# NVIDIAGameWorks/kaolin-wisp

Measured on AMD Instinct MI355X. Metric: training rays/sec, HashGrid NeRF (nerf_hash.yaml), synthetic Lego 800x800, higher is better.
Workload: dtype bf16

## Files before the change

### kaolin-wisp_amd/csrc/render.hip

```cpp
#include "wisp_common.h"
#include "raygen_dev.h"

#define WISP_DPP_ADD(V, CTRL, RMASK)                                                                                  \
    V += __builtin_bit_cast(float, __builtin_amdgcn_update_dpp(0, __builtin_bit_cast(int, V), CTRL, RMASK, 0xf, false))
static __device__ __forceinline__ float wave_incl_scan_f(float v, int ) {
    WISP_DPP_ADD(v, 0x111, 0xf);
    WISP_DPP_ADD(v, 0x112, 0xf);
    WISP_DPP_ADD(v, 0x114, 0xf);
    WISP_DPP_ADD(v, 0x118, 0xf);
    WISP_DPP_ADD(v, 0x142, 0xa);
    WISP_DPP_ADD(v, 0x143, 0xc);
    return v;
}
#undef WISP_DPP_ADD

static __device__ __forceinline__ float wave_last_f(float v) {
    return __builtin_bit_cast(float, __builtin_amdgcn_readlane(__builtin_bit_cast(int, v), 63));
}

static __device__ __forceinline__ float wave_sum_f(float v) { return wave_last_f(wave_incl_scan_f(v, 0)); }

__global__ void __launch_bounds__(256)
packed_sum_reduce_kernel(const float* __restrict__ feats, int64_t s_total, int channels,
                         const int64_t* __restrict__ pack_starts, int64_t num_packs, float* __restrict__ out) {
    const int lane = threadIdx.x & 63;
    const int64_t p = (int64_t)blockIdx.x * (blockDim.x >> 6) + (threadIdx.x >> 6);
    if (p >= num_packs) return;
    const int64_t b = pack_starts[p], e = (p + 1 < num_packs) ? pack_starts[p + 1] : s_total;
    for (int c = 0; c < channels; ++c) {
        float acc = 0.0f;
        for (int64_t i = b + lane; i < e; i += 64) acc += feats[i * channels + c];
        acc = wave_sum_f(acc);
        if (lane == 0) out[p * channels + c] = acc;
    }
}

__global__ void __launch_bounds__(256)
packed_cumsum_kernel(const float* __restrict__ feats, int64_t s_total, int channels,
                     const int64_t* __restrict__ pack_starts, int64_t num_packs, int exclusive, int reverse,
                     float* __restrict__ out) {
    const int lane = threadIdx.x & 63;
    const int64_t p = (int64_t)blockIdx.x * (blockDim.x >> 6) + (threadIdx.x >> 6);
    if (p >= num_packs) return;
    const int64_t b = pack_starts[p], e = (p + 1 < num_packs) ? pack_starts[p + 1] : s_total;
    const int64_t len = e - b;
    for (int c = 0; c < channels; ++c) {
        float carry = 0.0f;
        for (int64_t k0 = 0; k0 < len; k0 += 64) {
            const int64_t k = k0 + lane;
            const int64_t i = reverse ? (e - 1 - k) : (b + k);
            const float v = (k < len) ? feats[i * channels + c] : 0.0f;
            const float inc = wave_incl_scan_f(v, lane);
            if (k < len) out[i * channels + c] = carry + (exclusive ? inc - v : inc);
            carry += wave_last_f(inc);
        }
    }
}

extern "C" int wisp_packed_sum_reduce(const float* feats, int64_t num_samples, int channels, const int64_t* pack_starts,
                                      int64_t num_packs, float* out, wisp_stream_t stream) {
    WISP_REQUIRE(num_samples >= 0 && num_packs >= 0 && channels >= 1, "bad sizes");
    if (num_packs == 0) return WISP_OK;
    WISP_REQUIRE(feats && pack_starts && out, "null pointer");
    hipLaunchKernelGGL(packed_sum_reduce_kernel, dim3((unsigned)ceil_div64(num_packs, 4)), dim3(256), 0,
                       (hipStream_t)stream, feats, num_samples, channels, pack_starts, num_packs, out);
    WISP_CHECK_LAUNCH();
    return WISP_OK;
}

extern "C" int wisp_packed_cumsum(const float* feats, int64_t num_samples, int channels, const int64_t* pack_starts,
                                  int64_t num_packs, int exclusive, int reverse, float* out, wisp_stream_t stream) {
    WISP_REQUIRE(num_samples >= 0 && num_packs >= 0 && channels >= 1, "bad sizes");
    if (num_packs == 0) return WISP_OK;
    WISP_REQUIRE(feats && pack_starts && out, "null pointer");
    hipLaunchKernelGGL(packed_cumsum_kernel, dim3((unsigned)ceil_div64(num_packs, 4)), dim3(256), 0,
                       (hipStream_t)stream, feats, num_samples, channels, pack_starts, num_packs, exclusive, reverse, out);
    WISP_CHECK_LAUNCH();
    return WISP_OK;
}

struct Bg { float r, g, b; };

#define PACK_WAVES 1

__global__ void __launch_bounds__(256)
composite_init_kernel(int64_t num_rays, Bg bg, float* __restrict__ rgb, float* __restrict__ alpha,
                      float* __restrict__ depth, uint8_t* __restrict__ hit) {
    const int64_t r = (int64_t)blockIdx.x * blockDim.x + threadIdx.x;
    if (r >= num_rays) return;
    rgb[r * 3] = bg.r; rgb[r * 3 + 1] = bg.g; rgb[r * 3 + 2] = bg.b;
    alpha[r] = 0.0f;
    if (depth) depth[r] = 0.0f;
    hit[r] = 0;
}

template <bool BY_RAY>
__global__ void __launch_bounds__(256)
composite_fwd_kernel(const float* __restrict__ color, const float* __restrict__ density,
                     const float* __restrict__ deltas, const float* __restrict__ depths,
                     const int64_t* __restrict__ ridx, const int64_t* __restrict__ pack_starts, int64_t num_packs,
                     int64_t s_total, Bg bg, float* __restrict__ out_rgb, float* __restrict__ out_alpha,
                     float* __restrict__ out_depth, uint8_t* __restrict__ out_hit, float* __restrict__ weights) {
    const int lane = threadIdx.x & 63;
    const int64_t p = (int64_t)blockIdx.x * (blockDim.x >> 6) + (threadIdx.x >> 6);
    if (p >= num_packs) return;
    const int64_t b = pack_starts[p], e = (BY_RAY || p + 1 < num_packs) ? pack_starts[p + 1] : s_total;
    if (BY_RAY && b == e) {
        if (lane == 0) {
            out_alpha[p] = 0.0f; out_hit[p] = 0;
            out_rgb[p * 3] = bg.r; out_rgb[p * 3 + 1] = bg.g; out_rgb[p * 3 + 2] = bg.b;
            if (out_depth) out_depth[p] = 0.0f;
        }
        return;
    }
    float carry = 0.0f, sr = 0.0f, sg = 0.0f, sb = 0.0f, sa = 0.0f, sd = 0.0f;
    for (int64_t k0 = b; k0 < e; k0 += 64) {
        const int64_t i = k0 + lane;
        const bool live = i < e;
        const float tau = live ? density[i] * deltas[i] : 0.0f;
        const float inc = wave_incl_scan_f(tau, lane);
        const float excl = carry + (inc - tau);
        carry += wave_last_f(inc);
        if (live) {
            const float T = expf(-excl);
            const float w = T * (1.0f - expf(-tau));
            weights[i] = w;
            sr += w * color[i * 3]; sg += w * color[i * 3 + 1]; sb += w * color[i * 3 + 2];
            sa += w;
            if (depths) sd += w * depths[i];
        }
    }
    sr = wave_sum_f(sr); sg = wave_sum_f(sg); sb = wave_sum_f(sb); sa = wave_sum_f(sa);
    if (depths) sd = wave_sum_f(sd);
    if (lane == 0) {
        const int64_t r = BY_RAY ? p : ridx[b];
        out_alpha[r] = sa;
        out_hit[r] = sa > 0.0f ? 1 : 0;
        const float om = 1.0f - sa;
        out_rgb[r * 3] = bg.r * om + sr; out_rgb[r * 3 + 1] = bg.g * om + sg; out_rgb[r * 3 + 2] = bg.b * om + sb;
        if (out_depth) out_depth[r] = sd;
    }
}

template <bool BY_RAY>
__global__ void __launch_bounds__(256)
composite_bwd_kernel(const float* __restrict__ grad_rgb, const float* __restrict__ grad_alpha,
                     const float* __restrict__ grad_depth, const float* __restrict__ color,
                     const float* __restrict__ density, const float* __restrict__ deltas,
                     const float* __restrict__ depths, const int64_t* __restrict__ ridx,
                     const int64_t* __restrict__ pack_starts, int64_t num_packs, int64_t s_total, Bg bg,
                     float* __restrict__ grad_color, float* __restrict__ grad_density) {
    const int lane = threadIdx.x & 63;
    const int64_t p = (int64_t)blockIdx.x * (blockDim.x >> 6) + (threadIdx.x >> 6);
    if (p >= num_packs) return;
    const int64_t b = pack_starts[p], e = (BY_RAY || p + 1 < num_packs) ? pack_starts[p + 1] : s_total;
    if (BY_RAY && b == e) return;
    const int64_t r = BY_RAY ? p : ridx[b];
    const float gr = grad_rgb[r * 3], gg = grad_rgb[r * 3 + 1], gb = grad_rgb[r * 3 + 2];
    const float ga = grad_alpha ? grad_alpha[r] : 0.0f;
    const float gd = (grad_depth && depths) ? grad_depth[r] : 0.0f;
    float carry = 0.0f, tot = 0.0f;
    for (int64_t k0 = b; k0 < e; k0 += 64) {
        const int64_t i = k0 + lane;
        const bool live = i < e;
        const float tau = live ? density[i] * deltas[i] : 0.0f;
        const float inc = wave_incl_scan_f(tau, lane);
        const float excl = carry + (inc - tau);
        carry += wave_last_f(inc);
        if (live) {
            const float w = expf(-excl) * (1.0f - expf(-tau));
            float G = gr * (color[i * 3] - bg.r) + gg * (color[i * 3 + 1] - bg.g) + gb * (color[i * 3 + 2] - bg.b) + ga;
            if (depths) G += gd * depths[i];
            tot += G * w;
        }
    }
    tot = wave_sum_f(tot);
    carry = 0.0f;
    float gcarry = 0.0f;
    for (int64_t k0 = b; k0 < e; k0 += 64) {
        const int64_t i = k0 + lane;
        const bool live = i < e;
        const float dl = live ? deltas[i] : 0.0f;
        const float tau = live ? density[i] * dl : 0.0f;
        const float inc = wave_incl_scan_f(tau, lane);
        const float excl = carry + (inc - tau);
        carry += wave_last_f(inc);
        float T = 0.0f, et = 0.0f, w = 0.0f, G = 0.0f;
        if (live) {
            T = expf(-excl); et = expf(-tau); w = T * (1.0f - et);
            G = gr * (color[i * 3] - bg.r) + gg * (color[i * 3 + 1] - bg.g) + gb * (color[i * 3 + 2] - bg.b) + ga;
            if (depths) G += gd * depths[i];
        }
        const float gw = G * w;
        const float ginc = wave_incl_scan_f(gw, lane);
        const float suffix = tot - (gcarry + ginc);
        gcarry += wave_last_f(ginc);
        if (live) {
            grad_color[i * 3] = w * gr; grad_color[i * 3 + 1] = w * gg; grad_color[i * 3 + 2] = w * gb;
            grad_density[i] = (G * T * et - suffix) * dl;
        }
    }
}

extern "C" int wisp_composite_fwd(const float* color, const float* density, const float* deltas, const float* depths,
                                  const int64_t* ridx, const int64_t* pack_starts, int64_t num_packs,
                                  int64_t num_samples, int64_t num_rays, const float* bg, float* out_rgb,
                                  float* out_alpha, float* out_depth, uint8_t* out_hit, float* weights,
                                  wisp_stream_t stream) {
    WISP_REQUIRE(num_rays >= 0 && num_packs >= 0 && num_samples >= 0, "bad sizes");
    WISP_REQUIRE(bg, "null bg");
    if (num_rays == 0) return WISP_OK;
    WISP_REQUIRE(out_rgb && out_alpha && out_hit, "null output");
    WISP_REQUIRE(out_depth == nullptr || depths != nullptr, "out_depth needs depths");
    hipStream_t s = (hipStream_t)stream;
    const Bg b{bg[0], bg[1], bg[2]};
    if (ridx == nullptr) {
        WISP_REQUIRE(pack_starts && num_packs == num_rays, "ray-offset mode needs offsets[R+1] and num_packs == num_rays");
        WISP_REQUIRE(num_samples == 0 || (color && density && deltas && weights), "null pointer");
        hipLaunchKernelGGL(composite_fwd_kernel<true>, dim3((unsigned)ceil_div64(num_rays, PACK_WAVES)), dim3(64 * PACK_WAVES), 0, s, color,
                           density, deltas, out_depth ? depths : nullptr, ridx, pack_starts, num_rays, num_samples, b,
                           out_rgb, out_alpha, out_depth, out_hit, weights);
        WISP_CHECK_LAUNCH();
        return WISP_OK;
    }
    hipLaunchKernelGGL(composite_init_kernel, dim3((unsigned)ceil_div64(num_rays, 256)), dim3(256), 0, s, num_rays, b,
                       out_rgb, out_alpha, out_depth, out_hit);
    if (num_packs > 0) {
        WISP_REQUIRE(color && density && deltas && ridx && pack_starts && weights, "null pointer");
        hipLaunchKernelGGL(composite_fwd_kernel<false>, dim3((unsigned)ceil_div64(num_packs, 4)), dim3(256), 0, s, color,
                           density, deltas, out_depth ? depths : nullptr, ridx, pack_starts, num_packs, num_samples, b,
                           out_rgb, out_alpha, out_depth, out_hit, weights);
    }
    WISP_CHECK_LAUNCH();
    return WISP_OK;
}

extern "C" int wisp_composite_bwd(const float* grad_rgb, const float* grad_alpha, const float* grad_depth,
                                  const float* color, const float* density, const float* deltas, const float* depths,
                                  const int64_t* ridx, const int64_t* pack_starts, int64_t num_packs,
                                  int64_t num_samples, const float* bg, float* grad_color, float* grad_density,
                                  wisp_stream_t stream) {
    WISP_REQUIRE(num_packs >= 0 && num_samples >= 0 && bg, "bad sizes");
    if (num_packs == 0) return WISP_OK;
    WISP_REQUIRE(grad_rgb && color && density && deltas && pack_starts && grad_color && grad_density, "null pointer");
    const Bg b{bg[0], bg[1], bg[2]};
    if (ridx == nullptr)
        hipLaunchKernelGGL(composite_bwd_kernel<true>, dim3((unsigned)ceil_div64(num_packs, PACK_WAVES)), dim3(64 * PACK_WAVES), 0,
                           (hipStream_t)stream, grad_rgb, grad_alpha, grad_depth, color, density, deltas, depths, ridx,
                           pack_starts, num_packs, num_samples, b, grad_color, grad_density);
    else
        hipLaunchKernelGGL(composite_bwd_kernel<false>, dim3((unsigned)ceil_div64(num_packs, 4)), dim3(256), 0,
                           (hipStream_t)stream, grad_rgb, grad_alpha, grad_depth, color, density, deltas, depths, ridx,
                           pack_starts, num_packs, num_samples, b, grad_color, grad_density);
    WISP_CHECK_LAUNCH();
    return WISP_OK;
}

__global__ void __launch_bounds__(256)
find_depth_bound_kernel(int64_t num_packs, int64_t num_nugs, const float* __restrict__ query,
                        const int32_t* __restrict__ curr_in, int32_t* __restrict__ curr_out,
                        const float* __restrict__ depth) {
    const int64_t t = (int64_t)blockIdx.x * blockDim.x + threadIdx.x;
    if (t >= num_packs) return;
    int32_t result = -1;
    const int32_t start = curr_in[t];
    if (start > -1) {
        uint32_t i = (uint32_t)start;
        uint32_t stop = (t == num_packs - 1) ? (uint32_t)num_packs : (uint32_t)curr_in[t + 1];
        if ((int64_t)stop > num_nugs) stop = (uint32_t)num_nugs;
        const float q = query[t];
        while (i < stop) {
            const float entry = depth[2 * (int64_t)i], exit_ = depth[2 * (int64_t)i + 1];
            if ((q >= entry && q <= exit_) || q < entry) { result = (int32_t)i; break; }
            ++i;
        }
    }
    curr_out[t] = result;
}

extern "C" int wisp_find_depth_bound(const float* query, const int32_t* curr_idxes, const float* nug_depth,
                                     int64_t num_packs, int64_t num_nugs, int32_t* out, wisp_stream_t stream) {
    WISP_REQUIRE(num_packs >= 0 && num_nugs >= 0, "bad sizes");
    if (num_packs == 0) return WISP_OK;
    WISP_REQUIRE(query && curr_idxes && nug_depth && out, "null pointer");
    hipLaunchKernelGGL(find_depth_bound_kernel, dim3((unsigned)ceil_div64(num_packs, 256)), dim3(256), 0, (hipStream_t)stream,
                       num_packs, num_nugs, query, curr_idxes, out, nug_depth);
    WISP_CHECK_LAUNCH();
    return WISP_OK;
}

__global__ void __launch_bounds__(256)
sphere_trace_step_kernel(int64_t num_packs, const float* __restrict__ nug_o, const float* __restrict__ nug_d,
                         const float* __restrict__ nug_depth, const int32_t* __restrict__ nug_pidx, float dist_max,
                         float thr_close, float thr_avg, float* __restrict__ t, const float* __restrict__ dist, float* __restrict__ dist_prev,
                         uint8_t* __restrict__ mask, uint8_t* __restrict__ hit, const int32_t* __restrict__ curr_in,
                         int32_t* __restrict__ curr_out, int64_t* __restrict__ curr_pidx, float* __restrict__ x) {
#pragma clang fp contract(off)
    const int64_t p = (int64_t)blockIdx.x * blockDim.x + threadIdx.x;
    if (p >= num_packs) return;
    const int32_t cur = curr_in[p];
    bool m = mask[p] != 0;
    bool h = hit[p] != 0;
    const float dd = dist[p];
    float tt = t[p] + dd;
    if (m) {
        h = fabsf(dd) < thr_close;
        h = h || (fabsf(dd + dist_prev[p]) * 0.5f < thr_avg);
        m = tt < dist_max;
    }
    m = m && !h;
    if (m) dist_prev[p] = dd;
    int32_t nxt = -1;
    if (cur > -1) {
        uint32_t i = (uint32_t)cur;
        const uint32_t stop = (p == num_packs - 1) ? (uint32_t)num_packs : (uint32_t)curr_in[p + 1];
        while (i < stop) {
            const float entry = nug_depth[2 * (int64_t)i], exit_ = nug_depth[2 * (int64_t)i + 1];
            if ((tt >= entry && tt <= exit_) || tt < entry) { nxt = (int32_t)i; break; }
            ++i;
        }
    }
    m = m && (nxt != -1);
    const bool jumped = nxt != cur;
    const int32_t now = m ? nxt : cur;
    if (m && jumped) tt = nug_depth[2 * (int64_t)now];
    if (m) {
        x[p * 3 + 0] = nug_o[p * 3 + 0] + nug_d[p * 3 + 0] * tt;
        x[p * 3 + 1] = nug_o[p * 3 + 1] + nug_d[p * 3 + 1] * tt;
        x[p * 3 + 2] = nug_o[p * 3 + 2] + nug_d[p * 3 + 2] * tt;
        curr_pidx[p] = (int64_t)nug_pidx[now];
    } else if (mask[p] != 0) {
        x[p * 3 + 0] = nug_o[p * 3 + 0] + nug_d[p * 3 + 0] * tt;
        x[p * 3 + 1] = nug_o[p * 3 + 1] + nug_d[p * 3 + 1] * tt;
        x[p * 3 + 2] = nug_o[p * 3 + 2] + nug_d[p * 3 + 2] * tt;
    }
    t[p] = tt;
    mask[p] = m ? 1 : 0;
    hit[p] = h ? 1 : 0;
    curr_out[p] = now;
}

extern "C" int wisp_sphere_trace_step(int64_t num_packs, const float* nug_o, const float* nug_d, const float* nug_depth,
                                      const int32_t* nug_pidx, float dist_max, float thr_close, float thr_avg, float* t,
                                      const float* dist,
                                      float* dist_prev, uint8_t* mask, uint8_t* hit, const int32_t* curr_in,
                                      int32_t* curr_out, int64_t* curr_pidx, float* x, wisp_stream_t stream) {
    WISP_REQUIRE(num_packs >= 0, "negative count");
    if (num_packs == 0) return WISP_OK;
    WISP_REQUIRE(nug_o && nug_d && nug_depth && nug_pidx && t && dist && dist_prev && mask && hit && curr_in && curr_out &&
                 curr_pidx && x, "null pointer");
    hipLaunchKernelGGL(sphere_trace_step_kernel, dim3((unsigned)ceil_div64(num_packs, 256)), dim3(256), 0, (hipStream_t)stream,
                       num_packs, nug_o, nug_d, nug_depth, nug_pidx, dist_max, thr_close, thr_avg, t, dist, dist_prev, mask, hit, curr_in,
                       curr_out, curr_pidx, x);
    WISP_CHECK_LAUNCH();
    return WISP_OK;
}

template <bool ORTHO>
__global__ void __launch_bounds__(256)
raygen_kernel(const float* __restrict__ pixel_x, const float* __restrict__ pixel_y, int64_t n, RayCam cam,
              float* __restrict__ origins, float* __restrict__ dirs) {
    const int64_t i = (int64_t)blockIdx.x * blockDim.x + threadIdx.x;
    if (i >= n) return;
    float ow[3], dn[3];
    wisp_camera_ray<ORTHO>(pixel_x[i], pixel_y[i], cam, ow, dn);
#pragma unroll
    for (int c = 0; c < 3; ++c) {
        origins[i * 3 + c] = ow[c];
        dirs[i * 3 + c] = dn[c];
    }
}

extern "C" int wisp_generate_rays(const float* pixel_x, const float* pixel_y, int64_t num_pixels, int ortho, float x0,
                                  float y0, float width, float height, float scale_x, float scale_y,
                                  const float* view_rotation, const float* view_translation, float* origins, float* dirs,
                                  wisp_stream_t stream) {
    WISP_REQUIRE(num_pixels >= 0, "negative count");
    if (num_pixels == 0) return WISP_OK;
    WISP_REQUIRE(pixel_x && pixel_y && view_rotation && view_translation && origins && dirs, "null pointer");
    WISP_REQUIRE(width > 0.0f && height > 0.0f, "bad image size");
    RayCam cam;
    cam.x0 = x0; cam.y0 = y0; cam.width = width; cam.height = height; cam.sx = scale_x; cam.sy = scale_y;
    for (int k = 0; k < 9; ++k) cam.r[k] = view_rotation[k];
    for (int k = 0; k < 3; ++k) cam.t[k] = view_translation[k];
    const dim3 grid((unsigned)ceil_div64(num_pixels, 256));
    if (ortho)
        hipLaunchKernelGGL(raygen_kernel<true>, grid, dim3(256), 0, (hipStream_t)stream, pixel_x, pixel_y, num_pixels, cam, origins, dirs);
    else
        hipLaunchKernelGGL(raygen_kernel<false>, grid, dim3(256), 0, (hipStream_t)stream, pixel_x, pixel_y, num_pixels, cam, origins, dirs);
    WISP_CHECK_LAUNCH();
    return WISP_OK;
}

#define LOSS_BLOCKS 256
__global__ void __launch_bounds__(256)
rgb_loss_kernel(const float* __restrict__ rgb, const float* __restrict__ gt, int64_t n, int kind, float inv_n,
                float* __restrict__ grad, float* __restrict__ partial) {
    __shared__ float part[4];
    float acc = 0.0f;
    for (int64_t i = (int64_t)blockIdx.x * 256 + threadIdx.x; i < n; i += (int64_t)gridDim.x * 256) {
        const float x = rgb[i] - gt[i];
        float l, g;
        if (kind == 0) { const float a = fabsf(x); l = a < 1.0f ? 0.5f * x * x : a - 0.5f; g = fminf(fmaxf(x, -1.0f), 1.0f); }
        else if (kind == 1) { l = x * x; g = 2.0f * x; }
        else { l = fabsf(x); g = (x > 0.0f) ? 1.0f : (x < 0.0f ? -1.0f : 0.0f); }
        acc += l;
        grad[i] = g * inv_n;
    }
#pragma unroll
    for (int off = 32; off > 0; off >>= 1) acc += __shfl_down(acc, off, 64);
    if ((threadIdx.x & 63) == 0) part[threadIdx.x >> 6] = acc;
    __syncthreads();
    if (threadIdx.x == 0) partial[blockIdx.x] = (part[0] + part[1]) + (part[2] + part[3]);
}

__global__ void __launch_bounds__(1024)
loss_sum_kernel(const float* __restrict__ partial, int n, float inv_n, float* __restrict__ loss) {
    __shared__ float part[16];
    float t = 0.0f;
    for (int base = 0; base < n; base += 8 * 1024) {
        float v[8];
#pragma unroll
        for (int k = 0; k < 8; ++k) { const int i = base + threadIdx.x + k * 1024; v[k] = i < n ? partial[i] : 0.0f; }
#pragma unroll
        for (int k = 0; k < 8; ++k) t += v[k];
    }
#pragma unroll
    for (int off = 32; off > 0; off >>= 1) t += __shfl_down(t, off, 64);
    if ((threadIdx.x & 63) == 0) part[threadIdx.x >> 6] = t;
    __syncthreads();
    if (threadIdx.x == 0) {
        float s = 0.0f;
#pragma unroll
        for (int w = 0; w < 16; ++w) s += part[w];
        loss[0] = s * inv_n;
    }
}

extern "C" int wisp_rgb_loss(const float* rgb, const float* gt, int64_t num_elements, int kind, float* grad, float* loss,
                             float* workspace, wisp_stream_t stream) {
    WISP_REQUIRE(num_elements > 0 && rgb && gt && grad && loss && workspace, "bad arguments");
    WISP_REQUIRE(kind >= 0 && kind <= 2, "kind: 0 huber, 1 l2, 2 l1");
    const int blocks = (int)min64(ceil_div64(num_elements, 256), LOSS_BLOCKS);
    const float inv_n = 1.0f / (float)num_elements;
    hipLaunchKernelGGL(rgb_loss_kernel, dim3(blocks), dim3(256), 0, (hipStream_t)stream, rgb, gt, num_elements, kind, inv_n, grad,
                       workspace + 1);
    hipLaunchKernelGGL(loss_sum_kernel, dim3(1), dim3(1024), 0, (hipStream_t)stream, workspace + 1, blocks, inv_n, loss);
    WISP_CHECK_LAUNCH();
    return WISP_OK;
}

template <int W>
__global__ void __launch_bounds__(64 * W)
composite_loss_kernel(const float* __restrict__ color, const float* __restrict__ density, const float* __restrict__ deltas,
                      const int64_t* __restrict__ offsets, int64_t num_rays, int groups, Bg bg, const float* __restrict__ gt, int kind,
                      float inv_n, float* __restrict__ grad_color, float* __restrict__ grad_density, float* __restrict__ out_rgb,
                      float* __restrict__ partial) {
    const int lane = threadIdx.x & 63;
    const int v = blockIdx.x * W + (threadIdx.x >> 6);
    if (v >= groups) return;
    float lacc = 0.0f;
    for (int64_t r = v; r < num_rays; r += groups) {
        const int64_t b = offsets[r], e = offsets[r + 1];
        const float gt0 = gt[r * 3], gt1 = gt[r * 3 + 1], gt2 = gt[r * 3 + 2];
        const bool single = e - b <= 64;
        float carry = 0.0f, sr = 0.0f, sg = 0.0f, sb = 0.0f, sa = 0.0f;
        float dl = 0.0f, T = 0.0f, et = 0.0f, w = 0.0f, c0 = 0.0f, c1 = 0.0f, c2 = 0.0f;
        for (int64_t k0 = b; k0 < e; k0 += 64) {
            const int64_t i = k0 + lane;
            const bool live = i < e;
            dl = live ? deltas[i] : 0.0f;
            const float dn = live ? density[i] : 0.0f;
            c0 = live ? color[i * 3] : 0.0f; c1 = live ? color[i * 3 + 1] : 0.0f; c2 = live ? color[i * 3 + 2] : 0.0f;
            const float tau = live ? dn * dl : 0.0f;
            const float inc = wave_incl_scan_f(tau, lane);
            const float excl = carry + (inc - tau);
            carry += wave_last_f(inc);
            T = 0.0f; et = 0.0f; w = 0.0f;
            if (live) {
                T = expf(-excl); et = expf(-tau);
                w = T * (1.0f - et);
                sr += w * c0; sg += w * c1; sb += w * c2;
                sa += w;
            }
        }
        if (b < e) { sr = wave_sum_f(sr); sg = wave_sum_f(sg); sb = wave_sum_f(sb); sa = wave_sum_f(sa); }
        const float om = 1.0f - sa;
        const float rgb[3] = {bg.r * om + sr, bg.g * om + sg, bg.b * om + sb};
        const float gtc[3] = {gt0, gt1, gt2};
        float g[3], lsum[3];
#pragma unroll
        for (int c = 0; c < 3; ++c) {
            const float x = rgb[c] - gtc[c];
            float l, d;
            if (kind == 0) { const float a = fabsf(x); l = a < 1.0f ? 0.5f * x * x : a - 0.5f; d = fminf(fmaxf(x, -1.0f), 1.0f); }
            else if (kind == 1) { l = x * x; d = 2.0f * x; }
            else { l = fabsf(x); d = (x > 0.0f) ? 1.0f : (x < 0.0f ? -1.0f : 0.0f); }
            lsum[c] = l;
            g[c] = d * inv_n;
        }
        lacc += (lsum[0] + lsum[1]) + lsum[2];
        if (out_rgb && lane == 0) { out_rgb[r * 3] = rgb[0]; out_rgb[r * 3 + 1] = rgb[1]; out_rgb[r * 3 + 2] = rgb[2]; }
        if (b == e) continue;
        const float gr = g[0], gg = g[1], gb = g[2];
        if (single) {
            const int64_t i = b + lane;
            const bool live = i < e;
            const float G = live ? gr * (c0 - bg.r) + gg * (c1 - bg.g) + gb * (c2 - bg.b) : 0.0f;
            const float gw = G * w;
            const float ginc = wave_incl_scan_f(gw, lane);
            const float tot = wave_last_f(ginc);
            const float suffix = tot - ginc;
            if (live) {
                grad_color[i * 3] = w * gr; grad_color[i * 3 + 1] = w * gg; grad_color[i * 3 + 2] = w * gb;
                grad_density[i] = (G * T * et - suffix) * dl;
            }
            continue;
        }
        carry = 0.0f;
        float tot = 0.0f;
        for (int64_t k0 = b; k0 < e; k0 += 64) {
            const int64_t i = k0 + lane;
            const bool live = i < e;
            const float tau = live ? density[i] * deltas[i] : 0.0f;
            const float inc = wave_incl_scan_f(tau, lane);
            const float excl = carry + (inc - tau);
            carry += wave_last_f(inc);
            if (live) {
                const float ww = expf(-excl) * (1.0f - expf(-tau));
                const float G = gr * (color[i * 3] - bg.r) + gg * (color[i * 3 + 1] - bg.g) + gb * (color[i * 3 + 2] - bg.b);
                tot += G * ww;
            }
        }
        tot = wave_sum_f(tot);
        carry = 0.0f;
        float gcarry = 0.0f;
        for (int64_t k0 = b; k0 < e; k0 += 64) {
            const int64_t i = k0 + lane;
            const bool live = i < e;
            const float dd = live ? deltas[i] : 0.0f;
            const float tau = live ? density[i] * dd : 0.0f;
            const float inc = wave_incl_scan_f(tau, lane);
            const float excl = carry + (inc - tau);
            carry += wave_last_f(inc);
            float TT = 0.0f, ee = 0.0f, ww = 0.0f, G = 0.0f;
            if (live) {
                TT = expf(-excl); ee = expf(-tau); ww = TT * (1.0f - ee);
                G = gr * (color[i * 3] - bg.r) + gg * (color[i * 3 + 1] - bg.g) + gb * (color[i * 3 + 2] - bg.b);
            }
            const float gw = G * ww;
            const float ginc = wave_incl_scan_f(gw, lane);
            const float suffix = tot - (gcarry + ginc);
            gcarry += wave_last_f(ginc);
            if (live) {
                grad_color[i * 3] = ww * gr; grad_color[i * 3 + 1] = ww * gg; grad_color[i * 3 + 2] = ww * gb;
                grad_density[i] = (G * TT * ee - suffix) * dd;
            }
        }
    }
    if (lane == 0) partial[v] = lacc;
}

extern "C" int wisp_composite_loss(const float* color, const float* density, const float* deltas, const int64_t* ray_offsets,
                                   int64_t num_rays, int64_t num_samples, const float* bg, const float* gt, int kind,
                                   float* grad_color, float* grad_density, float* out_rgb, float* loss, float* workspace,
                                   int64_t workspace_floats, wisp_stream_t stream) {
    WISP_REQUIRE(num_rays > 0 && num_samples >= 0 && bg && gt && ray_offsets && loss && workspace && workspace_floats >= 1, "bad arguments");
    WISP_REQUIRE(kind >= 0 && kind <= 2, "kind: 0 huber, 1 l2, 2 l1");
    WISP_REQUIRE(num_samples == 0 || (color && density && deltas && grad_color && grad_density), "null pointer");
    const Bg b{bg[0], bg[1], bg[2]};
    const int groups = (int)min64(num_rays, min64(workspace_floats, (int64_t)1 << 22));
    const float inv_n = 1.0f / (float)(num_rays * 3);
    static const int waves = [] { const char* e = getenv("WISP_COMPOSITE_WAVES"); const int w = e ? atoi(e) : 4; return (w == 1 || w == 2) ? w : 4; }();
    if (waves == 1)
        hipLaunchKernelGGL(composite_loss_kernel<1>, dim3(groups), dim3(64), 0, (hipStream_t)stream, color, density, deltas, ray_offsets,
                           num_rays, groups, b, gt, kind, inv_n, grad_color, grad_density, out_rgb, workspace);
    else if (waves == 2)
        hipLaunchKernelGGL(composite_loss_kernel<2>, dim3((groups + 1) / 2), dim3(128), 0, (hipStream_t)stream, color, density, deltas, ray_offsets,
                           num_rays, groups, b, gt, kind, inv_n, grad_color, grad_density, out_rgb, workspace);
    else
        hipLaunchKernelGGL(composite_loss_kernel<4>, dim3((groups + 3) / 4), dim3(256), 0, (hipStream_t)stream, color, density, deltas, ray_offsets,
                           num_rays, groups, b, gt, kind, inv_n, grad_color, grad_density, out_rgb, workspace);
    hipLaunchKernelGGL(loss_sum_kernel, dim3(1), dim3(1024), 0, (hipStream_t)stream, workspace, groups, inv_n, loss);
    WISP_CHECK_LAUNCH();
    return WISP_OK;
}
```

Baseline: 13.42 million.

## Split long-ray compositing across four waves with shared-memory chunk scans

Result: faster. 13.60 million (median of 6 runs) (+1.3%).

```diff
diff --git a/kaolin-wisp_amd/csrc/render.hip b/kaolin-wisp_amd/csrc/render.hip
--- a/kaolin-wisp_amd/csrc/render.hip
+++ b/kaolin-wisp_amd/csrc/render.hip
@@ -561,6 +561,303 @@
     if (lane == 0) partial[v] = lacc;
 }
 
+#define WISP_DPP_ADD(V, CTRL, RMASK)                                                                                  \
+    V = V + __builtin_bit_cast(float, __builtin_amdgcn_update_dpp(0, __builtin_bit_cast(int, V), CTRL, RMASK, 0xf, false))
+static __device__ __forceinline__ float wave_incl_scan_prod_f(float a, float b) {
+#pragma clang fp contract(off)
+    const float p = a * b;
+    float v = fmaf(a, b, __builtin_bit_cast(float, __builtin_amdgcn_update_dpp(0, __builtin_bit_cast(int, p), 0x111, 0xf, 0xf, false)));
+    WISP_DPP_ADD(v, 0x112, 0xf);
+    WISP_DPP_ADD(v, 0x114, 0xf);
+    WISP_DPP_ADD(v, 0x118, 0xf);
+    WISP_DPP_ADD(v, 0x142, 0xa);
+    WISP_DPP_ADD(v, 0x143, 0xc);
+    return v;
+}
+#undef WISP_DPP_ADD
+
+static __device__ __forceinline__ float ray_loss_terms(float sr, float sg, float sb, float sa, const Bg& bg, float gt0, float gt1,
+                                                       float gt2, int kind, float inv_n, float (&rgb)[3], float (&g)[3]) {
+#pragma clang fp contract(off)
+    const float om = 1.0f - sa;
+    rgb[0] = fmaf(bg.r, om, sr); rgb[1] = fmaf(bg.g, om, sg); rgb[2] = fmaf(bg.b, om, sb);
+    const float gtc[3] = {gt0, gt1, gt2};
+    float lsum[3];
+#pragma unroll
+    for (int c = 0; c < 3; ++c) {
+        const float x = rgb[c] - gtc[c];
+        float l, d;
+        if (kind == 0) { const float a = fabsf(x); const float h = 0.5f * x; l = a < 1.0f ? h * x : a - 0.5f; d = fminf(fmaxf(x, -1.0f), 1.0f); }
+        else if (kind == 1) { l = x * x; d = 2.0f * x; }
+        else { l = fabsf(x); d = (x > 0.0f) ? 1.0f : (x < 0.0f ? -1.0f : 0.0f); }
+        lsum[c] = l;
+        g[c] = d * inv_n;
+    }
+    return (lsum[0] + lsum[1]) + lsum[2];
+}
+
+static __device__ __forceinline__ float composite_ray_serial(const float* __restrict__ color, const float* __restrict__ density,
+                                                             const float* __restrict__ deltas, int64_t b, int64_t e, int64_t r,
+                                                             int lane, const Bg& bg, const float* __restrict__ gt, int kind,
+                                                             float inv_n, float* __restrict__ grad_color,
+                                                             float* __restrict__ grad_density, float* __restrict__ out_rgb) {
+#pragma clang fp contract(off)
+    const float gt0 = gt[r * 3], gt1 = gt[r * 3 + 1], gt2 = gt[r * 3 + 2];
+    const bool single = e - b <= 64;
+    float carry = 0.0f, sr = 0.0f, sg = 0.0f, sb = 0.0f, sa = 0.0f;
+    float dl = 0.0f, T = 0.0f, et = 0.0f, w = 0.0f, c0 = 0.0f, c1 = 0.0f, c2 = 0.0f;
+    for (int64_t k0 = b; k0 < e; k0 += 64) {
+        const int64_t i = k0 + lane;
+        const bool live = i < e;
+        dl = live ? deltas[i] : 0.0f;
+        const float dn = live ? density[i] : 0.0f;
+        c0 = live ? color[i * 3] : 0.0f; c1 = live ? color[i * 3 + 1] : 0.0f; c2 = live ? color[i * 3 + 2] : 0.0f;
+        const float tau = live ? dn * dl : 0.0f;
+        const float inc = wave_incl_scan_f(tau, lane);
+        const float excl = carry + (inc - tau);
+        carry = carry + wave_last_f(inc);
+        T = 0.0f; et = 0.0f; w = 0.0f;
+        if (live) {
+            T = expf(-excl); et = expf(-tau);
+            w = (1.0f - et) * T;
+            sr = fmaf(c0, w, sr); sg = fmaf(c1, w, sg);
+            const float pb = c2 * w;
+            sb = sb + pb;
+            sa = sa + w;
+        }
+    }
+    if (b < e) { sr = wave_sum_f(sr); sg = wave_sum_f(sg); sb = wave_sum_f(sb); sa = wave_sum_f(sa); }
+    float rgb[3], g[3];
+    const float term = ray_loss_terms(sr, sg, sb, sa, bg, gt0, gt1, gt2, kind, inv_n, rgb, g);
+    if (out_rgb && lane == 0) { out_rgb[r * 3] = rgb[0]; out_rgb[r * 3 + 1] = rgb[1]; out_rgb[r * 3 + 2] = rgb[2]; }
+    if (b == e) return term;
+    const float gr = g[0], gg = g[1], gb = g[2];
+    if (single) {
+        const int64_t i = b + lane;
+        const bool live = i < e;
+        const float a0 = c0 - bg.r, a1 = c1 - bg.g, a2 = c2 - bg.b;
+        const float G = live ? fmaf(a2, gb, fmaf(a0, gr, a1 * gg)) : 0.0f;
+        const float ginc = wave_incl_scan_prod_f(w, G);
+        const float tot = wave_last_f(ginc);
+        const float suffix = tot - ginc;
+        if (live) {
+            grad_color[i * 3] = w * gr; grad_color[i * 3 + 1] = w * gg; grad_color[i * 3 + 2] = w * gb;
+            const float tg = T * G;
+            grad_density[i] = fmaf(et, tg, -suffix) * dl;
+        }
+        return term;
+    }
+    carry = 0.0f;
+    float tot = 0.0f;
+    for (int64_t k0 = b; k0 < e; k0 += 64) {
+        const int64_t i = k0 + lane;
+        const bool live = i < e;
+        const float tau = live ? density[i] * deltas[i] : 0.0f;
+        const float inc = wave_incl_scan_f(tau, lane);
+        const float excl = carry + (inc - tau);
+        carry = carry + wave_last_f(inc);
+        if (live) {
+            const float ww = (1.0f - expf(-tau)) * expf(-excl);
+            const float p0 = gr * (color[i * 3] - bg.r), p1 = gg * (color[i * 3 + 1] - bg.g), p2 = gb * (color[i * 3 + 2] - bg.b);
+            const float G = (p0 + p1) + p2;
+            tot = fmaf(ww, G, tot);
+        }
+    }
+    tot = wave_sum_f(tot);
+    carry = 0.0f;
+    float gcarry = 0.0f;
+    for (int64_t k0 = b; k0 < e; k0 += 64) {
+        const int64_t i = k0 + lane;
+        const bool live = i < e;
+        const float dd = live ? deltas[i] : 0.0f;
+        const float tau = live ? density[i] * dd : 0.0f;
+        const float inc = wave_incl_scan_f(tau, lane);
+        const float excl = carry + (inc - tau);
+        carry = carry + wave_last_f(inc);
+        float TT = 0.0f, ee = 0.0f, ww = 0.0f, G = 0.0f;
+        if (live) {
+            TT = expf(-excl); ee = expf(-tau); ww = (1.0f - ee) * TT;
+            const float p0 = gr * (color[i * 3] - bg.r), p2 = gb * (color[i * 3 + 2] - bg.b);
+            G = fmaf(gg, color[i * 3 + 1] - bg.g, p0) + p2;
+        }
+        const float ginc = wave_incl_scan_prod_f(ww, G);
+        const float suffix = tot - (gcarry + ginc);
+        gcarry = gcarry + wave_last_f(ginc);
+        if (live) {
+            grad_color[i * 3] = ww * gr; grad_color[i * 3 + 1] = ww * gg; grad_color[i * 3 + 2] = ww * gb;
+            const float tg = TT * G;
+            grad_density[i] = fmaf(ee, tg, -suffix) * dd;
+        }
+    }
+    return term;
+}
+
+template <int K>
+static __device__ __forceinline__ void chunk_carries(const float* tot, int nch, int wv, int lane, float (&out)[K]) {
+#pragma clang fp contract(off)
+    const float mine = lane < nch ? tot[lane] : 0.0f;
+    float run = 0.0f;
+#pragma unroll
+    for (int k = 0; k < K; ++k) {
+        out[k] = 0.0f;
+#pragma unroll
+        for (int q = 0; q < 4; ++q) {
+            if (q == wv) out[k] = run;
+            run = run + __builtin_bit_cast(float, __builtin_amdgcn_readlane(__builtin_bit_cast(int, mine), 4 * k + q));
+        }
+    }
+}
+
+template <int MODE>
+static __device__ __forceinline__ float chunk_accumulate(const float* sa, const float* sb, int nch, int lane) {
+#pragma clang fp contract(off)
+    float acc = 0.0f;
+    for (int cb = 0; cb < nch; cb += 4) {
+        float a[4], b[4];
+#pragma unroll
+        for (int q = 0; q < 4; ++q) { a[q] = MODE == 2 ? 0.0f : sa[(cb + q) * 64 + lane]; b[q] = sb[(cb + q) * 64 + lane]; }
+#pragma unroll
+        for (int q = 0; q < 4; ++q) {
+            if (cb + q < nch) {
+                if (MODE == 0) acc = fmaf(a[q], b[q], acc);
+                else if (MODE == 1) { const float p = a[q] * b[q]; acc = acc + p; }
+                else acc = acc + b[q];
+            }
+        }
+    }
+    return acc;
+}
+
+template <int K>
+__global__ void __launch_bounds__(256, 5)
+composite_loss_split_kernel(const float* __restrict__ color, const float* __restrict__ density, const float* __restrict__ deltas,
+                            const int64_t* __restrict__ offsets, int64_t num_rays, Bg bg, const float* __restrict__ gt, int kind,
+                            float inv_n, float* __restrict__ grad_color, float* __restrict__ grad_density,
+                            float* __restrict__ out_rgb, float* __restrict__ partial) {
+#pragma clang fp contract(off)
+    constexpr int NCH = 4 * K;
+    __shared__ float s_w[NCH * 64];
+    __shared__ float s_c[3][NCH * 64];
+    __shared__ float s_tot[NCH], s_gtot[NCH], s_sum[4];
+    const int lane = threadIdx.x & 63;
+    const int wv = threadIdx.x >> 6;
+    const int64_t r0 = (int64_t)blockIdx.x * 4;
+    int64_t ob[5];
+#pragma unroll
+    for (int j = 0; j < 5; ++j) ob[j] = offsets[r0 + j < num_rays ? r0 + j : num_rays];
+    {
+        const int64_t r = r0 + wv;
+        if (r < num_rays) {
+            const int64_t len = ob[wv + 1 < 5 ? wv + 1 : 4] - ob[wv];
+            const int64_t b = wv == 0 ? ob[0] : wv == 1 ? ob[1] : wv == 2 ? ob[2] : ob[3];
+            if (len <= 64 || len > 64 * NCH) {
+                float lacc = 0.0f;
+                lacc = lacc + composite_ray_serial(color, density, deltas, b, b + len, r, lane, bg, gt, kind, inv_n, grad_color,
+                                                   grad_density, out_rgb);
+                if (lane == 0) partial[r] = lacc;
+            }
+        }
+    }
+#pragma unroll 1
+    for (int j = 0; j < 4; ++j) {
+        const int64_t b = j == 0 ? ob[0] : j == 1 ? ob[1] : j == 2 ? ob[2] : ob[3];
+        const int64_t e = j == 0 ? ob[1] : j == 1 ? ob[2] : j == 2 ? ob[3] : ob[4];
+        const int64_t len = e - b;
+        if (len <= 64 || len > 64 * NCH) continue;
+        const int64_t r = r0 + j;
+        const int nch = (int)((len + 63) >> 6);
+        const float gt0 = gt[r * 3], gt1 = gt[r * 3 + 1], gt2 = gt[r * 3 + 2];
+        float dl[K], tau[K], inc[K], c0[K], c1[K], c2[K];
+#pragma unroll
+        for (int k = 0; k < K; ++k) {
+            const int64_t i = b + (int64_t)(wv + 4 * k) * 64 + lane;
+            const bool live = i < e;
+            dl[k] = live ? deltas[i] : 0.0f;
+            tau[k] = live ? density[i] : 0.0f;
+            c0[k] = live ? color[i * 3] : 0.0f; c1[k] = live ? color[i * 3 + 1] : 0.0f; c2[k] = live ? color[i * 3 + 2] : 0.0f;
+        }
+#pragma unroll
+        for (int k = 0; k < K; ++k) {
+            const int c = wv + 4 * k;
+            const bool live = b + (int64_t)c * 64 + lane < e;
+            tau[k] = live ? tau[k] * dl[k] : 0.0f;
+            inc[k] = wave_incl_scan_f(tau[k], lane);
+            if (c < nch && lane == 0) s_tot[c] = wave_last_f(inc[k]);
+        }
+        __syncthreads();
+        float T[K], et[K], w[K];
+        {
+            float carry[K];
+            chunk_carries<K>(s_tot, nch, wv, lane, carry);
+#pragma unroll
+            for (int k = 0; k < K; ++k) {
+                const int c = wv + 4 * k;
+                const bool live = b + (int64_t)c * 64 + lane < e;
+                const float excl = carry[k] + (inc[k] - tau[k]);
+                T[k] = 0.0f; et[k] = 0.0f; w[k] = 0.0f;
+                if (live) {
+                    T[k] = expf(-excl); et[k] = expf(-tau[k]);
+                    w[k] = (1.0f - et[k]) * T[k];
+                }
+                if (c < nch) {
+                    s_w[c * 64 + lane] = w[k];
+                    s_c[0][c * 64 + lane] = c0[k]; s_c[1][c * 64 + lane] = c1[k]; s_c[2][c * 64 + lane] = c2[k];
+                }
+            }
+        }
+        __syncthreads();
+        {
+            float acc;
+            if (wv == 0)      acc = chunk_accumulate<0>(s_c[0], s_w, nch, lane);
+            else if (wv == 1) acc = chunk_accumulate<0>(s_c[1], s_w, nch, lane);
+            else if (wv == 2) acc = chunk_accumulate<1>(s_c[2], s_w, nch, lane);
+            else              acc = chunk_accumulate<2>(s_w, s_w, nch, lane);
+            acc = wave_sum_f(acc);
+            if (lane == 0) s_sum[wv] = acc;
+        }
+        __syncthreads();
+        float rgb[3], g[3];
+        const float term = ray_loss_terms(s_sum[0], s_sum[1], s_sum[2], s_sum[3], bg, gt0, gt1, gt2, kind, inv_n, rgb, g);
+        if (wv == 0 && lane == 0) {
+            if (out_rgb) { out_rgb[r * 3] = rgb[0]; out_rgb[r * 3 + 1] = rgb[1]; out_rgb[r * 3 + 2] = rgb[2]; }
+            float lacc = 0.0f;
+            lacc = lacc + term;
+            partial[r] = lacc;
+        }
+        const float gr = g[0], gg = g[1], gb = g[2];
+        float G[K], ginc[K];
+#pragma unroll
+        for (int k = 0; k < K; ++k) {
+            const int c = wv + 4 * k;
+            const bool live = b + (int64_t)c * 64 + lane < e;
+            const int at = (c < nch ? c : 0) * 64 + lane;
+            const float a0 = s_c[0][at] - bg.r, a1 = s_c[1][at] - bg.g, a2 = s_c[2][at] - bg.b;
+            const float p0 = gr * a0, p1 = gg * a1, p2 = gb * a2;
+            const float Gt = live ? (p0 + p1) + p2 : 0.0f;
+            G[k] = live ? fmaf(gg, a1, p0) + p2 : 0.0f;
+            ginc[k] = wave_incl_scan_prod_f(w[k], G[k]);
+            if (c < nch) {
+                s_c[0][c * 64 + lane] = Gt;
+                if (lane == 0) s_gtot[c] = wave_last_f(ginc[k]);
+            }
+        }
+        __syncthreads();
+        const float tot = wave_sum_f(chunk_accumulate<0>(s_w, s_c[0], nch, lane));
+        float gcarry[K];
+        chunk_carries<K>(s_gtot, nch, wv, lane, gcarry);
+#pragma unroll
+        for (int k = 0; k < K; ++k) {
+            const int64_t i = b + (int64_t)(wv + 4 * k) * 64 + lane;
+            if (i < e) {
+                const float suffix = tot - (gcarry[k] + ginc[k]);
+                grad_color[i * 3] = w[k] * gr; grad_color[i * 3 + 1] = w[k] * gg; grad_color[i * 3 + 2] = w[k] * gb;
+                const float tg = T[k] * G[k];
+                grad_density[i] = fmaf(et[k], tg, -suffix) * dl[k];
+            }
+        }
+    }
+}
+
 extern "C" int wisp_composite_loss(const float* color, const float* density, const float* deltas, const int64_t* ray_offsets,
                                    int64_t num_rays, int64_t num_samples, const float* bg, const float* gt, int kind,
                                    float* grad_color, float* grad_density, float* out_rgb, float* loss, float* workspace,
@@ -572,7 +869,12 @@
     const int groups = (int)min64(num_rays, min64(workspace_floats, (int64_t)1 << 22));
     const float inv_n = 1.0f / (float)(num_rays * 3);
     static const int waves = [] { const char* e = getenv("WISP_COMPOSITE_WAVES"); const int w = e ? atoi(e) : 4; return (w == 1 || w == 2) ? w : 4; }();
-    if (waves == 1)
+    const char* se = getenv("WISP_COMPOSITE_SPLIT");
+    const bool split = waves == 4 && groups == num_rays && !(se && atoi(se) == 0);
+    if (split)
+        hipLaunchKernelGGL(composite_loss_split_kernel<4>, dim3((groups + 3) / 4), dim3(256), 0, (hipStream_t)stream, color, density, deltas,
+                           ray_offsets, num_rays, b, gt, kind, inv_n, grad_color, grad_density, out_rgb, workspace);
+    else if (waves == 1)
         hipLaunchKernelGGL(composite_loss_kernel<1>, dim3(groups), dim3(64), 0, (hipStream_t)stream, color, density, deltas, ray_offsets,
                            num_rays, groups, b, gt, kind, inv_n, grad_color, grad_density, out_rgb, workspace);
     else if (waves == 2)
```
